# brucechin/OctopusZK

Hardware: AMD Instinct MI355X
Metric: BN254 G1 VariableBaseMSM Mscalar-mul/s at 2^20 (higher is better)
Workload: dtype u32; 1 GPU; VariableBaseMSM BN254 G1 2^20 random scalars/bases per GPU, bit-exact vs the serial CPU path (BASELINE.json configs[1]); n_per_gpu=1048576, window_bits=16, windows=8, glv=True, prepared_bases=False, msms_in_flight=3, schedule=pipeline3, parallelism=index-range shard x1, RCCL all-gather of 192-B partials + HIP point sum

## Files before the change

### include/ozk.h

```cpp
#ifndef OZK_H
#define OZK_H

#include <stddef.h>
#include <stdint.h>

#ifdef __cplusplus
extern "C" {
#endif

#define OZK_OK 0
#define OZK_E_INVALID -1
#define OZK_E_NO_DEVICE -2
#define OZK_E_NOMEM -3
#define OZK_E_INTERNAL -4

#define OZK_G1 1
#define OZK_G2 2

const char* ozk_last_error(void);
int ozk_version(void);
int ozk_device_count(void);
int ozk_device_cu_count(void);
int ozk_stream_create_cu_range(int32_t first_cu, int32_t n_cus, void** stream);
int ozk_stream_destroy(void* stream);
// ... 33 lines not shown
                            size_t* accum_ws_bytes);
int ozk_var_msm_sort_dev(const void* d_bases, int32_t prepared, const void* d_scalars, int32_t n, int32_t type,
                         void* d_sorted, size_t sorted_bytes, void* d_sort_ws, size_t sort_ws_bytes, void* stream);
int ozk_var_msm_accum_dev(const void* d_prepared, int32_t n, int32_t type, void* d_sorted, size_t sorted_bytes,
                          void* d_accum_ws, size_t accum_ws_bytes, void* d_tail, size_t tail_bytes, void* stream,
                          int32_t part);

size_t ozk_var_msm_prepared_bytes(int32_t n, int32_t type);
int ozk_var_msm_prepare_dev(const void* d_bases, int32_t n, int32_t type, void* d_prepared, size_t prepared_size,
                            void* stream);
int ozk_var_msm_prepared_dev(const void* d_prepared, const void* d_scalars, int32_t n, int32_t type, void* d_out,
                             void* d_workspace, size_t workspace_bytes, void* stream);
int ozk_bases_create_host(const uint8_t* bases, int32_t n, int32_t type, int32_t task_id, void** handle);
int ozk_var_msm_bases_host(void* handle, const uint8_t* scalars, int32_t n, uint8_t* out);
int ozk_bases_destroy(void* handle);
int ozk_bases_type(void* handle);

int ozk_order_event_create(void** ev);
int ozk_order_event_destroy(void* ev);


int ozk_points_sum_dev(const void* d_points, int32_t k, int32_t type, void* d_out, void* stream);

int ozk_groth16_combine_dev(const void* d_records, int32_t world, void* d_proof, void* stream);

int ozk_prof_enable(int on);
int ozk_prof_dominant_kernel_ms(double* avg_ms, int* launches);
int ozk_prof_dominant_kernel_stats(double* stats4, int* launches);
int ozk_prof_dominant_kernel_clock_mhz(double* stats4, int* launches);
double ozk_prof_clock_khz(void);
int ozk_var_msm_plan(int32_t n, int32_t* window_bits, int32_t* windows);
int ozk_var_msm_glv(int32_t n);
int ozk_var_msm_last_l1_path(void);

int ozk_gen_bases_dev(uint64_t seed, int32_t n, int32_t type, void* d_out_wire, void* stream);

int ozk_fixed_batch_msm_host(int32_t outerc, int32_t window_size, int32_t out_len,
                             int32_t inner_len, int32_t n, int32_t scalar_size,
                             const uint8_t* base, const uint8_t* scalars, int32_t bn_type,
                             int32_t task_id, uint8_t* out);
int ozk_fixed_double_batch_msm_host(int32_t outerc1, int32_t window_size1, int32_t outerc2,
                                    int32_t window_size2, int32_t out_len1, int32_t inner_len1,
                                    int32_t out_len2, int32_t inner_len2, int32_t n,
                                    const uint8_t* base_g1, const uint8_t* base_g2,
                                    const uint8_t* scalars, int32_t task_id, uint8_t* out);
int ozk_field_batch_mul_host(const uint8_t* in, int32_t n, int32_t task_id, uint8_t* out);

size_t ozk_fixed_batch_msm_workspace_bytes(int32_t outerc, int32_t window_size, int32_t n,
                                           int32_t bn_type);
int ozk_fixed_batch_msm_dev(int32_t outerc, int32_t window_size, int32_t n, const void* d_base,
                            const void* d_scalars, int32_t bn_type, void* d_out,
                            void* d_workspace, size_t workspace_bytes, void* stream);
int ozk_field_batch_mul_dev(const void* d_in, int32_t n, void* d_out, void* stream);
int ozk_fixed_batch_msm_compact_dev(int32_t outerc, int32_t window_size, int32_t n, const void* d_base,
                                    const void* d_scalars, int32_t bn_type, void* d_out, void* d_workspace,
                                    size_t workspace_bytes, void* stream);
int ozk_fixed_batch_msm_compact_host(int32_t outerc, int32_t window_size, int32_t n, const uint8_t* base,
                                     const uint8_t* scalars, int32_t bn_type, int32_t task_id, uint8_t* out);
int ozk_fixed_batch_msm_base_dev(int32_t outerc, int32_t window_size, int32_t n, const uint8_t* base_host,
                                 const void* d_scalars, int32_t bn_type, void* d_out, int32_t compact,
                                 void* d_workspace, size_t workspace_bytes, void* stream);

int ozk_fft_host(const uint8_t* in, int32_t n, const uint8_t* omega, int32_t task_id,
                 uint8_t* out);
size_t ozk_fft_workspace_bytes(int32_t n);
int ozk_fft_dev(const void* d_in, int32_t n, const uint8_t* omega_host32, void* d_out,
// ... 118 lines not shown
```

### octopuszk_amd/build.py

```python
import os
import shutil
import subprocess
import sys

HERE = os.path.dirname(os.path.abspath(__file__))
CSRC = os.path.join(HERE, "csrc")
ROOT = os.path.dirname(HERE)
LIB = os.path.join(HERE, "libozk_hip.so")

HIP_SOURCES = ["msm_var.hip", "msm_var_g2.hip", "msm_fixed.hip", "fft.hip", "host_ctx.hip", "pairing.hip", "msm_multi.hip",
               "point_codec.hip", "points_scale.hip", "ec_fft.hip", "points_mul.hip"]
HEADERS = ["consts_gen.h", "mad_chain_gen.h", "fp29.cuh", "fq2.cuh", "fq12.cuh", "batch_verify.cuh", "point_codec.cuh", "points_scale.cuh", "points_mul.cuh", "ec_fft.cuh", "bace.cuh", "kzg.cuh", "kzg_set.cuh", "pairing_consts_gen.h", "ec.cuh", "quad.cuh", "curve.cuh", "msm_var.cuh", "msm_var_driver.cuh", "msm_multi.cuh", "glv.cuh", "l1_whole.h", "ozk_common.h", "knobs.h", "host_ctx.h", "pin_cache.h",
           os.path.join("..", "..", "include", "ozk.h")]
HIPCC_FLAGS = ["-std=c++17", "-O3", "--offload-arch=gfx950", "-fPIC", "-fno-gpu-rdc", "-Wno-unused-result",
               "-Wno-pass-failed"]

JNI_LIBS = {
    "libAlgebraMSMVariableBaseMSM.so": "jni_var_msm.c",
    "libAlgebraMSMFixedBaseMSM.so": "jni_fixed_msm.c",
    "libAlgebraFFTAuxiliary.so": "jni_fft.c",
}


def _newer(target, deps):
    if not os.path.exists(target):
        return True
    t = os.path.getmtime(target)
    return any(os.path.exists(d) and os.path.getmtime(d) > t for d in deps)


def hipcc():
    for cand in (shutil.which("hipcc"), "/opt/rocm/bin/hipcc"):
        if cand and os.path.exists(cand):
            return cand
    raise RuntimeError("hipcc not found: the HIP library cannot be built (there is no CPU path)")


def build(force=False, verbose=True):
    srcs = [os.path.join(CSRC, s) for s in HIP_SOURCES if os.path.exists(os.path.join(CSRC, s))]
    deps = srcs + [os.path.join(CSRC, h) for h in HEADERS]
    if force or _newer(LIB, deps):
        defs = []
        if os.path.exists(os.path.join(CSRC, "fq2.cuh")):
            defs.append("-DOZK_WITH_G2")
        objdir = os.path.join(HERE, "_obj")
# ... 38 lines not shown
```

### octopuszk_amd/csrc/ec.cuh

```cuda
#pragma once
#include "fp29.cuh"

namespace ozk {

template <class EA>
struct Aff {
  EA x, y;
};

template <class CV>
struct Jac {
  typename CV::EX X;
  typename CV::EY Y;
  typename CV::EZ Z;
};

template <class CV>
OZK_HD bool is_inf(const Jac<CV>& p) { return is_zero(p.Z); }

template <class EA>
OZK_HD bool is_inf(const Aff<EA>& q) { return is_zero(q.x) && is_zero(q.y); }

template <class CV>
OZK_HD Jac<CV> from_affine(const Aff<typename CV::EA>& q) {
// ... 178 lines not shown
    Aff<typename CV::EA> qs = q;
    qs.y = typename CV::EA(reduce_to<17>(normalise(yq)));
    return xyzz_from_affine<CV>(qs);
  }
  const auto U2 = mul(q.x, p.ZZ);
  const auto S2 = mul(yq, p.ZZZ);
  const auto P = sub(U2, p.X);
  const auto R = sub(S2, p.Y);
  const auto PP = sqr(P);
  if (is_zero(PP)) {
    if (is_zero(R)) {
      Aff<typename CV::EA> qs = q;
      qs.y = typename CV::EA(reduce_to<17>(normalise(yq)));
      return xyzz_dbl_affine<CV>(qs);
    }
    Xyzz<CV> z = p;
    z.ZZ = typename CV::XZZ(el_zero(q.x));
    z.ZZZ = typename CV::XZZZ(el_zero(q.x));
    return z;
  }
  const auto PPP = mul(P, PP);
  const auto Q = mul(p.X, PP);
  const auto X3 = sub_sub2(sqr(R), PPP, Q);
  const auto Y3 = mul2(sub_nc(Q, X3), R, neg_nc(p.Y), PPP);
  Xyzz<CV> out;
  out.X = typename CV::XX(X3);
  out.Y = typename CV::XY(Y3);
  out.ZZ = typename CV::XZZ(mul(p.ZZ, PP));
  out.ZZZ = typename CV::XZZZ(mul(p.ZZZ, PPP));
  return out;
}

template <class CV>
OZK_HD Xyzz<CV> xyzz_dbl(const Xyzz<CV>& p) {
  if (is_inf(p)) return p;
  const auto U = dbl(p.Y);
  const auto V = sqr(U);
  const auto W = mul(U, V);
  const auto S = mul(p.X, V);
  const auto xx = sqr(p.X);
  const auto M = add(dbl(xx), xx);
  const auto X3 = sub(sqr(M), dbl(S));
  const auto Y3 = mulsub(M, sub(S, X3), W, p.Y);
  Xyzz<CV> r;
  r.X = typename CV::XX(X3);
  r.Y = typename CV::XY(Y3);
  r.ZZ = typename CV::XZZ(mul(V, p.ZZ));
  r.ZZZ = typename CV::XZZZ(mul(W, p.ZZZ));
  return r;
}

template <class CV>
OZK_HD Xyzz<CV> xyzz_add(const Xyzz<CV>& p, const Xyzz<CV>& q) {
  if (is_inf(q)) return p;
  if (is_inf(p)) return q;
  const auto U1 = mul(p.X, q.ZZ);
  const auto U2 = mul(q.X, p.ZZ);
  const auto S1 = mul(p.Y, q.ZZZ);
  const auto S2 = mul(q.Y, p.ZZZ);
  const auto P = sub(U2, U1);
  const auto R = sub(S2, S1);
  if (is_zero(P)) {
    if (is_zero(R)) return xyzz_dbl(p);
    Xyzz<CV> z = p;
    z.ZZ = typename CV::XZZ(el_zero(p.ZZ));
    z.ZZZ = typename CV::XZZZ(el_zero(p.ZZ));
    return z;
  }
  const auto PP = sqr(P);
  const auto PPP = mul(P, PP);
  const auto Q = mul(U1, PP);
  const auto X3 = sub(sqr(R), add(PPP, dbl(Q)));
  const auto Y3 = mulsub(R, sub(Q, X3), S1, PPP);
  Xyzz<CV> out;
  out.X = typename CV::XX(X3);
  out.Y = typename CV::XY(Y3);
  out.ZZ = typename CV::XZZ(mul(mul(p.ZZ, q.ZZ), PP));
  out.ZZZ = typename CV::XZZZ(mul(mul(p.ZZZ, q.ZZZ), PPP));
  return out;
}

template <class CV>
OZK_HD Jac<CV> xyzz_to_jac(const Xyzz<CV>& p) {
  Jac<CV> r;
  r.X = typename CV::EX(mul(p.X, p.ZZ));
  r.Y = typename CV::EY(mul(p.Y, p.ZZZ));
  r.Z = typename CV::EZ(p.ZZ);
  return r;
}

template <class CV>
OZK_HD Jac<CV> jac_add(const Jac<CV>& p, const Jac<CV>& q) {
  if (is_inf(p)) return q;
  if (is_inf(q)) return p;
  const auto& X1 = p.X;
  const auto& Y1 = p.Y;
  const auto& X2 = q.X;
  const auto& Y2 = q.Y;
  const auto Z1 = entry_reduce<32, CV>(p.Z);
  const auto Z2 = entry_reduce<32, CV>(q.Z);
  const auto Z1Z1 = sqr(Z1);
  const auto Z2Z2 = sqr(Z2);
  const auto U1 = mul(X1, Z2Z2);
  const auto U2 = mul(X2, Z1Z1);
  const auto S1 = mul(mul(Y1, Z2), Z2Z2);
  const auto S2 = mul(mul(Y2, Z1), Z1Z1);
  const auto H = sub(U2, U1);
  const auto rh = sub(S2, S1);
  if (is_zero(H)) {
    if (is_zero(rh)) return jac_dbl(p);
    return jac_infinity<CV>();
  }
  const auto I = sqr(dbl(H));
  const auto J = mul(H, I);
  const auto r = dbl(rh);
  const auto V = mul(U1, I);
  const auto X3 = sub(sqr(r), add(J, dbl(V)));
  const auto Y3 = mulsub(r, sub(V, X3), dbl(S1), J);
  const auto Z3 = mul(sub(sqr(add(Z1, Z2)), add(Z1Z1, Z2Z2)), H);
  Jac<CV> out;
// ... 42 lines not shown
```

### octopuszk_amd/csrc/fp29.cuh

```cuda
#pragma once
#include "consts_gen.h"
#include <type_traits>

#if defined(__HIPCC__)
#include <hip/hip_runtime.h>
#define OZK_HD __host__ __device__ __forceinline__
#else
#define OZK_HD inline
#endif

namespace ozk {

constexpr int ceil_div(long long a, long long b) { return (int)((a + b - 1) / b); }
constexpr int MONT_SLACK = 169;
constexpr int FE_BMAX = 16 * FE_MAXK;

template <class P, int B>
struct Fe {
  static_assert(B >= 1 && B <= FE_BMAX, "bound out of range");
  u32 l[9];
  OZK_HD Fe() {}
  template <int B2, class = std::enable_if_t<(B2 <= B)>>
  OZK_HD Fe(const Fe<P, B2>& o) {
#pragma unroll
// ... 371 lines not shown
  static_assert(B >= 1 && B <= FE_BMAX, "bound out of range");
  static_assert(LU >= 2 && LU <= 15, "limb bound out of range");
  u32 l[9];
  OZK_HD FeL() {}
  OZK_HD FeL(const Fe<P, B>& o) {
#pragma unroll
    for (int i = 0; i < 9; i++) l[i] = o.l[i];
  }
};
template <class P, int B, int LU>
OZK_HD Fe<P, B> normalise(const FeL<P, B, LU>& a) {
  Fe<P, B> r;
#pragma unroll
  for (int i = 0; i < 9; i++) r.l[i] = a.l[i];
  fe_carry(r);
  return r;
}
template <class P, int B2>
OZK_HD auto neg_nc(const Fe<P, B2>& b) {
  constexpr int K = B2 / 16 + 1;
  static_assert(K <= FE_MAXK, "sub bias table too small");
  FeL<P, neg_bound(B2), 4> r;
#pragma unroll
  for (int i = 0; i < 9; i++) r.l[i] = P::BIAS[K][i] - b.l[i];
  return r;
}
template <class P, int B1, int B2>
OZK_HD auto sub_nc(const Fe<P, B1>& a, const Fe<P, B2>& b) {
  constexpr int K = B2 / 16 + 1;
  static_assert(K <= FE_MAXK, "sub bias table too small");
  FeL<P, B1 + 16 * K, 6> r;
#pragma unroll
  for (int i = 0; i < 9; i++) r.l[i] = a.l[i] + (P::BIAS[K][i] - b.l[i]);
  return r;
}
template <class P, int B1, int B2, int B3>
OZK_HD auto sub_sub2(const Fe<P, B1>& a, const Fe<P, B2>& b, const Fe<P, B3>& c) {
  constexpr int K2 = B2 / 16 + 1, K3 = B3 / 16 + 1;
  static_assert(K2 <= FE_MAXK && K3 <= FE_MAXK, "sub bias table too small");
  Fe<P, B1 + 16 * K2 + 32 * K3> r;
#pragma unroll
  for (int i = 0; i < 9; i++) r.l[i] = a.l[i] + (P::BIAS[K2][i] - b.l[i]) + ((P::BIAS[K3][i] - c.l[i]) << 1);
  fe_carry(r);
  return r;
}
template <class P, int B1, int LU1, int B2>
OZK_HD auto select_el(bool c, const FeL<P, B1, LU1>& a, const Fe<P, B2>& b) {
  FeL<P, (B1 > B2 ? B1 : B2), LU1> r;
#pragma unroll
  for (int i = 0; i < 9; i++) r.l[i] = c ? a.l[i] : b.l[i];
  return r;
}
template <class P, int B1, int LU, int B2>
OZK_HD auto mul(const FeL<P, B1, LU>& a, const Fe<P, B2>& b) {
  static_assert(LU <= 12, "loose factor too wide for the 64-bit column accumulator");
  Fe<P, B1> an;
#pragma unroll
  for (int i = 0; i < 9; i++) an.l[i] = a.l[i];
  return mul(an, b);
}
template <class P, int B1, int LU1, int B2, int B3, int LU3, int B4>
OZK_HD auto mul2(const FeL<P, B1, LU1>& a, const Fe<P, B2>& b, const FeL<P, B3, LU3>& c, const Fe<P, B4>& d) {
  static_assert(LU1 + LU3 <= 12, "loose factors too wide for the 64-bit column accumulator");
  Fe<P, B1> an;
  Fe<P, B3> cn;
#pragma unroll
// ... 326 lines not shown
```

### octopuszk_amd/csrc/knobs.h

```cpp
#pragma once
#include <stdlib.h>
#include <string.h>

#include <atomic>
#include <mutex>

namespace ozk {

constexpr int KNOB_COMPUTED = -0x7fffffff;
constexpr int KNOB_STRING = KNOB_COMPUTED + 1;

#define OZK_KNOBS(X)                                                                                                     \
                                                   \
  X(MSM_GLV, "OZK_MSM_GLV", 1, "0: plain 256-bit windows instead of the GLV split (var MSM up to 2^23 pairs, fixed base)") \
  X(MSM_SIGNED, "OZK_MSM_SIGNED", 1, "0: unsigned window digits in the GLV form")                                        \
  X(MSM_C, "OZK_MSM_C", KNOB_COMPUTED, "window bits, 1..16 (default: the cost model's choice)")                          \
  X(MSM_L1, "OZK_MSM_L1", KNOB_COMPUTED, "sorted entries per level-1 lane (default: from the bucket size; 0 as unset)")   \
  X(MSM_L1_WHOLE, "OZK_MSM_L1_WHOLE", 1, "G1 level 1 by whole buckets on lane groups: 0 never, 1 on every plan that can take it (unset: where it pays)") \
  X(MSM_L1_ROUNDS, "OZK_MSM_L1_ROUNDS", 2, "most rounds of resident workgroups level 1 is rounded up to; 0: no rounding") \
  X(MSM_TAIL_MODE, "OZK_MSM_TAIL_MODE", -1, "0 / 1: force the latency / throughput shape of the window sums")            \
  X(MSM_SMALL_SORT, "OZK_MSM_SMALL_SORT", 1, "0: small MSMs take the two-level sort too")                                \
  X(MSM_S_LAT, "OZK_MSM_S_LAT", KNOB_COMPUTED, "buckets per lane in a latency tail's fused first level (default: 8 G1, 4 G2)") \
  X(MSM_FIN_MAX, "OZK_MSM_FIN_MAX", 4, "elements per window left to the final one-wave kernel, 1..16")                   \
                                                                                                    \
  X(HOST_SLICES, "OZK_HOST_SLICES", 8, "most slices a host-buffer MSM is cut into; 1: no slicing")                       \
  X(HOST_SLICE_MIN_LOG, "OZK_HOST_SLICE_MIN_LOG", 18, "log2 of the smallest slice")                                      \
  X(SHARD, "OZK_SHARD", 0, "1: the JNI entries shard large calls over the visible devices")                              \
  X(SHARD_MIN_N, "OZK_SHARD_MIN_N", 1 << 21, "smallest call OZK_SHARD=1 shards")                                         \
  X(SHARD_COUNT, "OZK_SHARD_COUNT", 0, "shards of such a call; 0: one per device")                                       \
  X(SHARD_RCCL, "OZK_SHARD_RCCL", 1, "0: the partials of a sharded call go through the host, not RCCL")                  \
  X(COPY_HELPERS, "OZK_COPY_HELPERS", 3, "threads staging host buffers beside the caller, 0..11 (first use only)")       \
  X(HOST_TRACE, "OZK_HOST_TRACE", 0, "1: per-call host timings on stderr; 2: with absolute timestamps")                  \
                                                                                     \
  X(FB_WS, "OZK_FB_WS", KNOB_COMPUTED, "window bits of a GLV fixed-base table (default: cost model, at most the caller's)") \
  X(FB_AFFINE, "OZK_FB_AFFINE", 1, "0: Jacobian gather-add instead of affine table records")                             \
  X(FB_TABLE_CACHE, "OZK_FB_TABLE_CACHE", 1, "0: window tables are built per call")                                      \
  X(FB_TABLE_CACHE_MB, "OZK_FB_TABLE_CACHE_MB", 1024, "MiB of cached window tables per device")                          \
  X(FB_TABLE_CACHE_SECOND_USE, "OZK_FB_TABLE_CACHE_SECOND_USE", 1, "0: a table is cached on its first use")              \
  X(FB_HOST_RANGES, "OZK_FB_HOST_RANGES", 4, "ranges a host fixed-base call downloads its results in")                   \
  X(MM_WS, "OZK_MM_WS", KNOB_COMPUTED, "window bits of the shared-base batched MSM (default: from n)")                   \
                                                                                             \
  X(FFT_MAXK, "OZK_FFT_MAXK", 8, "most butterfly stages per pass, 3..10")                                                \
  X(FFT_PLAN, "OZK_FFT_PLAN", 1, "0: stages spread evenly over the passes")                                              \
  X(FFT_KS, "OZK_FFT_KS", KNOB_STRING, "explicit stages per pass, e.g. \"8,6,8\" (must sum to log2 n)")                  \
  X(FFT_TW_PYRAMID, "OZK_FFT_TW_PYRAMID", 1, "0: twiddles from the flat table")                                          \
  X(FFT_PLAN_CACHE, "OZK_FFT_PLAN_CACHE", 1, "0: twiddle tables are built per call")                                     \
  X(FFT_PLAN_CACHE_MB, "OZK_FFT_PLAN_CACHE_MB", 4096, "MiB of cached twiddle tables per device")                         \
  X(QAP_FOLD_SCALE, "OZK_QAP_FOLD_SCALE", 1, "0: the witness map scales in a pass of its own")                           \
  X(BACE_LDS_SLOTS, "OZK_BACE_LDS_SLOTS", 16, "circuit slots kept in LDS, 0..28")

enum Knob {
#define X(id, env, dflt, doc) K_##id,
  OZK_KNOBS(X)
// ... 56 lines not shown
```

### octopuszk_amd/csrc/msm_var.cuh

```cuda
#pragma once
#include "curve.cuh"
#include "glv.cuh"
#include "l1_whole.h"

namespace ozk {

constexpr u32 BID_NONE = 0xffffffffu;

struct MsmPlan {
  int n_in;
  int glv;
  int n;
  int sd;
  int c;
  int cb;
  int W;
  int L1;
  int LK;
  int S;
  int lone;
  int small_sort;
  int S_lat;
  int fin_max;
  int tail_mode;
  int l1_whole;
  int l1_gtop;
};

OZK_HD u32 scalar_digit(const u32 (&s)[8], int w, int c) {
  const int bit = w * c;
  const int wi = bit >> 5, sh = bit & 31;
  u32 v = s[wi] >> sh;
  if (sh + c > 32 && wi + 1 < 8) v |= s[wi + 1] << (32 - sh);
  return v & ((1u << c) - 1u);
}

OZK_HD bool digit_decode(u32 code, int sd, u32& b, u32& neg) {
  if (sd) {
    const u32 t = code - 1u;
    b = t >> 1;
    neg = t & 1u;
  } else {
    b = code;
    neg = 0;
  }
  return code != 0;
}
template <class Emit>
OZK_HD void signed_digit_codes(const u32 (&e)[8], int c, int W, bool neg, Emit emit) {
  const u32 half = 1u << (c - 1);
  const u32 thr = (c == 16 && neg) ? half - 1u : half;
  u32 cy = 0;
  for (int w = 0; w < W; w++) {
    const u32 d = scalar_digit(e, w, c) + cy;
    cy = d > thr;
    const u32 m = cy ? (1u << c) - d : d;
    emit(w, (uint16_t)(m ? (((m - 1u) << 1) | (cy ^ (u32)neg)) + 1u : 0u));
// ... 1128 lines not shown
  b.ZZZ = ElemTraits<typename CV::XZZZ>::load_raw(w + 3 * RW);
  return b;
}

template <class CV>
__global__ void __launch_bounds__(256)
k_l1_whole(const uint4* __restrict__ items, const uint2* __restrict__ sent, const u32* __restrict__ pts_in,
           const u32* __restrict__ bad, WholeGeom geo, u32 n_lanes, u32* __restrict__ buckets,
           unsigned long long* __restrict__ clk) {
  using IO = CurveIO<CV>;
  using Acc = RunAcc<CV, true>;
  if (*bad != 0u) return;
  unsigned long long w0 = 0, c0 = 0;
  if (clk != nullptr && threadIdx.x == 0) {
    w0 = (unsigned long long)wall_clock64();
    c0 = (unsigned long long)clock64();
    atomicMax(&clk[0], ~w0);
  }
  const u32 t = blockIdx.x * blockDim.x + threadIdx.x;
  u32 item, g, G;
  whole_lane_map(geo, t < n_lanes ? t : 0u, &item, &g, &G);
  const bool valid = t < n_lanes && item != WHOLE_NO_ITEM;
  uint4 it = items[valid ? item : 0u];
  if (!valid) it.y = 0u;
  u32 first, n_e;
  whole_part(it.y, g, G, &first, &n_e);
  Xyzz<CV> a = xyzz_from_affine<CV>(IO::aff_infinity());
  if (n_e != 0u) {
    const u32* idx_c = reinterpret_cast<const u32*>(sent + (size_t)it.x + first);
    u32 v_cur = idx_c[0];
    u32 v_next = idx_c[n_e > 1u ? 2 : 0];
    const __amdgpu_buffer_rsrc_t table = Acc::table_rsrc(pts_in);
    typename Acc::Raw r = Acc::load_raw_buf(table, v_cur);
    for (u32 k = 0; k < n_e; k++) {
      const bool negate = (v_cur & SIDX_NEG) != 0;
      const auto q = Acc::decode_unsigned(r);
      const u32 k2 = (k + 2 < n_e) ? k + 2 : n_e - 1;
      r = Acc::load_raw_buf(table, v_next);
      v_cur = v_next;
      v_next = idx_c[2 * (size_t)k2];
      a = xyzz_madd_lazy(a, q, negate);
    }
  }
  if (__ballot(G > 1u) != 0ull) {
    const Xyzz<CV> b = xyzz_quad_swap<0xB1, CV>(a);
    if (G > 1u) a = xyzz_add(a, b);
  }
  if (__ballot(G > 2u) != 0ull) {
    const Xyzz<CV> b = xyzz_quad_swap<0x4E, CV>(a);
    if (G > 2u) a = xyzz_add(a, b);
  }
  if (g == 0u && it.y != 0u) IO::store_rec_xyzz(a, buckets + (size_t)it.z * IO::REC_WORDS);
  if (clk != nullptr && (threadIdx.x & 63) == 0) {
    const unsigned long long w1 = (unsigned long long)wall_clock64();
    atomicMax(&clk[1], w1);
    if (threadIdx.x == 0) {
      atomicAdd(&clk[2], (unsigned long long)clock64() - c0);
      atomicAdd(&clk[3], w1 - w0);
    }
  }
}

template <class CV, bool FIRSTLEVEL>
__global__ void __launch_bounds__(256)
k_wsum(const u32* __restrict__ A_in, const u32* __restrict__ R_in, const u32* __restrict__ hist,
       int m_in, int S, int g, u32* __restrict__ A_out, u32* __restrict__ R_out, int m_out, int W, int prio) {
  using IO = CurveIO<CV>;
  if (prio) __builtin_amdgcn_s_setprio(3);
  const int t = blockIdx.x * blockDim.x + threadIdx.x;
  if (t >= m_out * W) return;
  const int w = t / m_out, j = t - w * m_out;
  const size_t base = (size_t)w * m_in;
  const int lo = j * S;
// ... 66 lines not shown
  wave_combine<CV>(A, T, l, valid, g);
  if (l == 0) {
    IO::store_jac(A, A_out + ((size_t)w * m_out + j) * IO::JAC_WORDS);
    IO::store_jac(T, R_out + ((size_t)w * m_out + j) * IO::JAC_WORDS);
  }
}

template <class CV>
__global__ void __launch_bounds__(64)
k_wsum_fused(const u32* __restrict__ buckets, const u32* __restrict__ hist, int m_in, int S, int sg,
             u32* __restrict__ A_out, u32* __restrict__ R_out, int m_out, int W, int prio) {
  using IO = CurveIO<CV>;
  if (prio) __builtin_amdgcn_s_setprio(3);
  const int wave = blockIdx.x;
  if (wave >= m_out * W) return;
  const int w = wave / m_out, j = wave - w * m_out;
  const int l = threadIdx.x & 63;
  const int nseg = (m_in + S - 1) / S;
  int valid = nseg - j * 64;
  if (valid > 64) valid = 64;
  const size_t base = (size_t)w * m_in;
  const int lo = (j * 64 + l) * S;
  int hi = lo + S;
  if (hi > m_in) hi = m_in;
  Jac<CV> run = jac_infinity<CV>(), ws = jac_infinity<CV>();
  for (int e = hi - 1; e >= lo; e--) {
    if (hist[base + e] != 0) run = jac_add(run, IO::load_rec(buckets + (base + e) * IO::REC_WORDS));
    if (e > lo) ws = jac_add(ws, run);
  }
  wave_combine<CV>(ws, run, l, valid, sg);
  if (l == 0) {
    IO::store_jac(ws, A_out + ((size_t)w * m_out + j) * IO::JAC_WORDS);
    IO::store_jac(run, R_out + ((size_t)w * m_out + j) * IO::JAC_WORDS);
  }
}

struct SliceBuckets {
  const u32* buckets[16];
  const u32* hist[16];
};
template <class CV>
__global__ void __launch_bounds__(256) k_bucket_combine(SliceBuckets t, int K, u32* __restrict__ buckets0,
                                                        u32* __restrict__ hist0, size_t NB) {
  using IO = CurveIO<CV>;
  const size_t e = (size_t)blockIdx.x * blockDim.x + threadIdx.x;
  if (e >= NB) return;
  bool have = hist0[e] != 0, changed = false;
  Jac<CV> acc = jac_infinity<CV>();
  if (have) acc = IO::load_rec(buckets0 + e * IO::REC_WORDS);
  for (int k = 1; k < K; k++) {
    if (t.hist[k][e] == 0) continue;
    acc = jac_add(acc, IO::load_rec(t.buckets[k] + e * IO::REC_WORDS));
    changed = true;
  }
  if (changed) {
    IO::store_rec_jac(acc, buckets0 + e * IO::REC_WORDS);
    hist0[e] = 1;
  }
}

template <class CV>
__device__ __forceinline__ void write_normalised_inline(const Jac<CV>& r, u32* out) {
  CurveIO<CV>::template write<WireOut>(r, out);
}
template <class CV>
__device__ void write_normalised(const Jac<CV>& r, u32* out) {
// ... 140 lines not shown
```

### octopuszk_amd/csrc/msm_var.hip

```cpp
#include "msm_var_driver.cuh"

#include <dlfcn.h>
#include <rccl/rccl.h>

#include <algorithm>
#include <chrono>
#include <new>
#include <string>
#include <thread>
#include <vector>

OZK_G2_DRIVER_INSTANCES(extern)

using namespace ozk;

template <class F>
static auto with_plan(int n, int type, F f) {
  return by_point_type(type, [&](auto t) { return f(t, plan_for<typename decltype(t)::CV>(n, false)); });
}
#define CV_OF(t) typename decltype(t)::CV

extern "C" {

size_t ozk_var_msm_workspace_bytes(int32_t n, int32_t type) {
// ... 743 lines not shown
  *launches = (int)m.size();
  if (m.empty()) return OZK_OK;
  std::sort(m.begin(), m.end());
  stats4[0] = tot / (double)m.size();
  stats4[1] = m[m.size() / 2];
  stats4[2] = m.front();
  stats4[3] = m.back();
  return OZK_OK;
}

double ozk_prof_clock_khz(void) { return g_prof.clk_khz; }

int ozk_var_msm_plan(int32_t n, int32_t* window_bits, int32_t* windows) {
  if (n <= 0 || !window_bits || !windows) return fail(OZK_E_INVALID, "bad argument");
  const MsmPlan p = make_plan(n);
  *window_bits = p.c;
  *windows = p.W;
  return OZK_OK;
}

int ozk_var_msm_glv(int32_t n) { return n > 0 ? make_plan(n).glv : 0; }

int ozk_var_msm_last_l1_path(void) {
  const L1PathLast& last = g_l1_path_last;
  if (last.planned <= 0) return last.planned;
  u32 bad = 0;
  if (hipDeviceSynchronize() != hipSuccess || hipMemcpy(&bad, last.d_bad, sizeof(bad), hipMemcpyDeviceToHost) != hipSuccess) {
    (void)hipGetLastError();
    return -1;
  }
  return bad ? 0 : 1;
}

const char* ozk_last_error(void) { return err_buf(); }
int ozk_version(void) { return 2; }
int ozk_device_count(void) {
  int n = 0;
  if (hipGetDeviceCount(&n) != hipSuccess) return 0;
  return n;
}

}
```

### octopuszk_amd/csrc/msm_var_driver.cuh

```cuda
#pragma once
#include <hip/hip_ext.h>
#include <pthread.h>
#include <stdlib.h>

#include <atomic>
#include <vector>

#include "msm_var.cuh"
#include "host_ctx.h"
#include "fq2.cuh"

namespace ozk {

enum { PROF_OFF = 0, PROF_EVENTS = 1, PROF_CLOCK = 2 };
struct ProfState {
  pthread_mutex_t mu = PTHREAD_MUTEX_INITIALIZER;
  std::atomic<int> mode{PROF_OFF};
  int src = PROF_EVENTS;
  int every = 1, seen = 0;
  int count = 0;
  std::vector<hipEvent_t> e0, e1;
  bool created = false;
  int ev_device = -1;
  unsigned long long* d_clk = nullptr;
// ... 73 lines not shown
  p.sd = sd_ok && c >= 2;
  p.cb = c - p.sd;
  p.W = ((p.glv ? 128 : 256) + c - 1) / c;
  {
    const long long per_bucket = (long long)p.n >> p.cb;
    long long l1 = per_bucket * 5 / 16;
    long long l1_min = p.n >= (1 << 20) ? 52 : 40;
    if (p.glv) {
      const long long cap = (long long)p.n * p.W;
      long long fit = cap / 65536;
      const int top_bits = 127 - (p.W - 1) * p.c;
      const int tb = top_bits - p.sd;
      const long long per_top = (top_bits >= 1 && top_bits < p.c) ? ((long long)p.n >> (tb > 0 ? tb : 0)) : per_bucket;
      const long long pieces = (per_top + 9) / 10;
      if (fit < pieces) fit = pieces;
      if (fit < 8) fit = 8;
      if (fit < l1_min) l1_min = fit;
    }
    if (l1 < l1_min) l1 = l1_min;
    if (l1 > 1024) l1 = 1024;
    p.L1 = knob_or(K_MSM_L1, (int)l1);
  }
  if (p.L1 < 2) p.L1 = 2;
  p.LK = PLAN_LK;
  p.S = PLAN_S;
  p.lone = 0;
  p.small_sort = p.n <= SORTS_MAX_N && p.cb <= SORTS_MAX_CB && knob(K_MSM_SMALL_SORT) != 0;
  p.S_lat = p.S;
  p.fin_max = knob(K_MSM_FIN_MAX);
  if (p.fin_max < 1) p.fin_max = 1;
  if (p.fin_max > 16) p.fin_max = 16;
  p.tail_mode = knob(K_MSM_TAIL_MODE);
  if (p.tail_mode != 0 && p.tail_mode != 1) p.tail_mode = -1;
  p.l1_whole = 0;
  p.l1_gtop = WHOLE_G;
  return p;
}

template <class CV>
static MsmPlan plan_for(int n, bool lone) {
  MsmPlan p = make_plan(n);
  p.lone = lone;
  const long long max_rounds = knob(K_MSM_L1_ROUNDS);
  bool rounded = false;
  if ((CV::LDS_ACC || lone) && knob_or(K_MSM_L1, 0) == 0 && max_rounds != 0) {
    static int cu_count = 0;
    if (cu_count == 0) {
      int dev = 0, cus = 0;
      if (hipGetDevice(&dev) == hipSuccess && hipDeviceGetAttribute(&cus, hipDeviceAttributeMultiprocessorCount, dev) == hipSuccess &&
          cus > 0)
        cu_count = cus;
      else
        cu_count = 256;
    }
    const int slots = (CV::LDS_ACC ? 2 : 3) * cu_count;
    const long long cap = (long long)p.n * p.W;
    const long long blocks = ((cap + p.L1 - 1) / p.L1 + 255) / 256;
    long long rounds = blocks / slots > 0 ? blocks / slots : 1;
    if (rounds > max_rounds) rounds = max_rounds;
    long long l1 = (cap + 256LL * slots * rounds - 1) / (256LL * slots * rounds);
    if (l1 > p.L1 && l1 <= 1024) {
      p.L1 = (int)l1;
      rounded = true;
    }
  }
  const int s_lat = knob_or(K_MSM_S_LAT, std::is_same<CV, G1Cfg>::value && p.cb >= 13 ? 8 : p.S);
// ... 285 lines not shown
    lanes = (n_in + p.LK - 1) / p.LK;
    if (!first_generic && (int)lanes <= SMALL_LEVEL_LANES) {
      hipLaunchKernelGGL((k_segreduce_small<CT>), dim3(1), dim3(TB), 0, st, L.total + 1, (int)n_in, p.LK, L.buckets,
                         L.slot_bid[cur], L.slot_pts[cur], L.slot_bid[cur ^ 1], L.slot_pts[cur ^ 1]);
      break;
    }
    hipLaunchKernelGGL((k_segreduce<CT, false>), dim3((unsigned)((lanes + TB - 1) / TB)), dim3(TB), 0, st,
                       first_generic ? L.slot_bid2 : L.slot_bid[cur], (const u32*)nullptr, L.slot_pts[cur],
                       L.total + 1, (int)n_in, p.LK, L.buckets, L.slot_bid[cur ^ 1], L.slot_pts[cur ^ 1], (int)lanes,
                       (unsigned long long*)nullptr);
    first_generic = false;
    if (lanes == 1) break;
    n_in = 2 * lanes;
    cur ^= 1;
  }
  OZK_HIP(hipGetLastError());
  return OZK_OK;
}

template <class CV>
int var_msm_head(const MsmPlan& p, const void* d_bases, const void* d_scalars, void* ws, size_t ws_bytes, void* tail,
                        size_t tail_bytes, hipStream_t st, hipEvent_t order_ev = nullptr,
                        const void* prepared = nullptr) {
  const RegionBytes rb = region_bytes<CV>(p);
  if (rb.sorted + rb.sort_ws + rb.accum_ws > ws_bytes)
    return fail(OZK_E_INVALID, "workspace too small: need %zu bytes, got %zu", rb.sorted + rb.sort_ws + rb.accum_ws,
                ws_bytes);
  uint8_t* w = (uint8_t*)ws;
  int rc = var_msm_sort<CV>(p, d_bases, d_scalars, w, rb.sorted, w + rb.sorted, rb.sort_ws, st, order_ev, prepared);
  if (rc) return rc;
  return var_msm_accum<CV>(p, w, rb.sorted, w + rb.sorted + rb.sort_ws, rb.accum_ws, tail, tail_bytes, st, prepared);
}

template <class CV>
int var_msm_tail(const MsmPlan& p, void* tail, size_t tail_bytes, void* d_out, hipStream_t st,
                        hipEvent_t order_ev = nullptr, int mode = TAIL_LATENCY) {
  hip_clear_stale();
  using CT = CV;
  MsmLayout L;
  const size_t tneed = tail_layout<CV>(p, L, tail, tail_bytes);
  if (tneed > tail_bytes) return fail(OZK_E_INVALID, "tail buffer too small: need %zu bytes, got %zu", tneed, tail_bytes);
  const int shape = p.tail_mode >= 0 ? p.tail_mode : mode;
  const bool fused = shape == TAIL_LATENCY;
  const int S0 = fused && mode == TAIL_LATENCY ? p.S_lat : p.S;
  launch_wsum0<CV>(p, L, st, S0, fused);
  int m_in, g, k = 0;
  first_level_shape(p, S0, fused, &m_in, &g);
  const int TB = 256;
  const int sg = ilog2((uint32_t)p.S);
  while (shape == TAIL_THROUGHPUT && m_in > TAIL_SERIAL_ABOVE) {
    const int m_out = (m_in + p.S - 1) / p.S;
    const int tot = m_out * p.W;
    hipLaunchKernelGGL((k_wsum<CT, false>), dim3((tot + TB - 1) / TB), dim3(TB), 0, st, L.wA[k], L.wR[k],
                       (const u32*)nullptr, m_in, p.S, g, L.wA[k ^ 1], L.wR[k ^ 1], m_out, p.W, 1);
    m_in = m_out;
    g += sg;
    k ^= 1;
  }
  if (order_ev) OZK_HIP(hipEventRecord(order_ev, st));
  while (m_in > p.fin_max) {
    const int m_out = (m_in + 63) / 64;
    const int tot = m_out * p.W;
    hipLaunchKernelGGL((k_wsum_wave<CT>), dim3(tot), dim3(64), 0, st, L.wA[k], L.wR[k], m_in, g, L.wA[k ^ 1],
                       L.wR[k ^ 1], m_out, p.W);
    m_in = m_out;
    g += 6;
    k ^= 1;
  }
  hipLaunchKernelGGL((k_finalize<CT>), dim3(1), dim3(64), 0, st, L.wA[k], L.wR[k], m_in, g, p.W, p.c, p.sd,
                     (u32*)d_out);
  OZK_HIP(hipGetLastError());
  return OZK_OK;
}

template <class CV>
// ... 273 lines not shown
```

### octopuszk_amd/lib.py

```python
import ctypes
import os

HERE = os.path.dirname(os.path.abspath(__file__))
LIB_PATH = os.environ.get("OZK_LIB_PATH") or os.path.join(HERE, "libozk_hip.so")

_lib = None

c_u8p = ctypes.POINTER(ctypes.c_uint8)
i32 = ctypes.c_int32
vp = ctypes.c_void_p
sz = ctypes.c_size_t

_SIGS = {
    "ozk_last_error": (ctypes.c_char_p, []),
    "ozk_version": (ctypes.c_int, []),
    "ozk_device_count": (ctypes.c_int, []),
    "ozk_var_msm_host": (ctypes.c_int, [vp, vp, i32, i32, i32, vp]),
    "ozk_var_double_msm_host": (ctypes.c_int, [vp, vp, vp, i32, i32, vp]),
    "ozk_var_msm_sharded_host": (ctypes.c_int, [vp, vp, i32, i32, i32, vp]),
    "ozk_var_msm_auto_host": (ctypes.c_int, [vp, vp, i32, i32, i32, vp]),
    "ozk_var_double_msm_sharded_host": (ctypes.c_int, [vp, vp, vp, i32, i32, vp]),
    "ozk_var_double_msm_auto_host": (ctypes.c_int, [vp, vp, vp, i32, i32, vp]),
    "ozk_shard_last_exchange": (ctypes.c_int, []),
    "ozk_shard_comms_release": (None, []),
    "ozk_var_msm_workspace_bytes": (sz, [i32, i32]),
    "ozk_var_msm_dev": (ctypes.c_int, [vp, vp, i32, i32, vp, vp, sz, vp]),
    "ozk_prof_enable": (ctypes.c_int, [ctypes.c_int]),
    "ozk_prof_dominant_kernel_ms": (ctypes.c_int, [ctypes.POINTER(ctypes.c_double), ctypes.POINTER(ctypes.c_int)]),
    "ozk_prof_dominant_kernel_stats": (ctypes.c_int, [ctypes.POINTER(ctypes.c_double), ctypes.POINTER(ctypes.c_int)]),
    "ozk_prof_clock_khz": (ctypes.c_double, []),
    "ozk_prof_dominant_kernel_clock_mhz": (ctypes.c_int, [ctypes.POINTER(ctypes.c_double), ctypes.POINTER(ctypes.c_int)]),
    "ozk_var_msm_plan": (ctypes.c_int, [i32, ctypes.POINTER(i32), ctypes.POINTER(i32)]),
    "ozk_var_msm_glv": (ctypes.c_int, [i32]),
    "ozk_var_msm_last_l1_path": (ctypes.c_int, []),
    "ozk_gen_bases_dev": (ctypes.c_int, [ctypes.c_uint64, i32, i32, vp, vp]),
    "ozk_var_msm_stage_bytes": (ctypes.c_int, [i32, i32, ctypes.POINTER(sz), ctypes.POINTER(sz), ctypes.POINTER(sz)]),
    "ozk_var_msm_sort_dev": (ctypes.c_int, [vp, i32, vp, i32, i32, vp, sz, vp, sz, vp]),
    "ozk_var_msm_accum_dev": (ctypes.c_int, [vp, i32, i32, vp, sz, vp, sz, vp, sz, vp, i32]),
    "ozk_device_cu_count": (ctypes.c_int, []),
    "ozk_stream_create_cu_range": (ctypes.c_int, [i32, i32, ctypes.POINTER(ctypes.c_void_p)]),
    "ozk_stream_destroy": (ctypes.c_int, [vp]),
    "ozk_var_msm_head_workspace_bytes": (sz, [i32, i32]),
    "ozk_var_msm_tail_bytes": (sz, [i32, i32]),
    "ozk_var_msm_head_dev": (ctypes.c_int, [vp, i32, vp, i32, i32, vp, sz, vp, sz, vp, vp]),
    "ozk_var_msm_tail_dev": (ctypes.c_int, [i32, i32, vp, sz, vp, vp, vp, i32]),
    "ozk_bases_create_host": (ctypes.c_int, [vp, i32, i32, i32, ctypes.POINTER(vp)]),
    "ozk_var_msm_bases_host": (ctypes.c_int, [vp, vp, i32, vp]),
    "ozk_bases_destroy": (ctypes.c_int, [vp]),
    "ozk_var_msm_prepared_bytes": (sz, [i32, i32]),
    "ozk_var_msm_prepare_dev": (ctypes.c_int, [vp, i32, i32, vp, sz, vp]),
    "ozk_var_msm_prepared_dev": (ctypes.c_int, [vp, vp, i32, i32, vp, vp, sz, vp]),
    "ozk_order_event_create": (ctypes.c_int, [ctypes.POINTER(vp)]),
    "ozk_order_event_destroy": (ctypes.c_int, [vp]),
    "ozk_points_sum_dev": (ctypes.c_int, [vp, i32, i32, vp, vp]),
    "ozk_groth16_combine_dev": (ctypes.c_int, [vp, i32, vp, vp]),
    "ozk_fixed_batch_msm_host": (ctypes.c_int, [i32, i32, i32, i32, i32, i32, vp, vp, i32, i32, vp]),
    "ozk_fixed_double_batch_msm_host": (ctypes.c_int, [i32] * 9 + [vp, vp, vp, i32, vp]),
    "ozk_field_batch_mul_host": (ctypes.c_int, [vp, i32, i32, vp]),
    "ozk_fixed_batch_msm_workspace_bytes": (sz, [i32, i32, i32, i32]),
    "ozk_fixed_batch_msm_dev": (ctypes.c_int, [i32, i32, i32, vp, vp, i32, vp, vp, sz, vp]),
    "ozk_field_batch_mul_dev": (ctypes.c_int, [vp, i32, vp, vp]),
    "ozk_fixed_batch_msm_compact_dev": (ctypes.c_int, [i32, i32, i32, vp, vp, i32, vp, vp, sz, vp]),
    "ozk_fixed_batch_msm_compact_host": (ctypes.c_int, [i32, i32, i32, vp, vp, i32, i32, vp]),
    "ozk_fixed_batch_msm_base_dev": (ctypes.c_int, [i32, i32, i32, vp, vp, i32, vp, i32, vp, sz, vp]),
    "ozk_fft_compact_host": (ctypes.c_int, [vp, i32, vp, i32, vp]),
    "ozk_fft_compact_dev": (ctypes.c_int, [vp, i32, vp, vp, vp, sz, vp]),
    "ozk_tuning_reload": (ctypes.c_int, []),
# ... 98 lines not shown
```

Baseline: 742.6 Mscalar-mul/s.

## Add row/column window-sum tail and cheaper first bucket additions

Result: faster. 751.4 Mscalar-mul/s, median of 6 (+1.2%).

```diff
diff --git a/include/ozk.h b/include/ozk.h
--- a/include/ozk.h
+++ b/include/ozk.h
@@ -89,6 +89,7 @@
 int ozk_var_msm_plan(int32_t n, int32_t* window_bits, int32_t* windows);
 int ozk_var_msm_glv(int32_t n);
 int ozk_var_msm_last_l1_path(void);
+int ozk_var_msm_last_tail_form(void);
 
 int ozk_gen_bases_dev(uint64_t seed, int32_t n, int32_t type, void* d_out_wire, void* stream);
 
diff --git a/octopuszk_amd/build.py b/octopuszk_amd/build.py
--- a/octopuszk_amd/build.py
+++ b/octopuszk_amd/build.py
@@ -10,7 +10,7 @@
 
 HIP_SOURCES = ["msm_var.hip", "msm_var_g2.hip", "msm_fixed.hip", "fft.hip", "host_ctx.hip", "pairing.hip", "msm_multi.hip",
                "point_codec.hip", "points_scale.hip", "ec_fft.hip", "points_mul.hip"]
-HEADERS = ["consts_gen.h", "mad_chain_gen.h", "fp29.cuh", "fq2.cuh", "fq12.cuh", "batch_verify.cuh", "point_codec.cuh", "points_scale.cuh", "points_mul.cuh", "ec_fft.cuh", "bace.cuh", "kzg.cuh", "kzg_set.cuh", "pairing_consts_gen.h", "ec.cuh", "quad.cuh", "curve.cuh", "msm_var.cuh", "msm_var_driver.cuh", "msm_multi.cuh", "glv.cuh", "l1_whole.h", "ozk_common.h", "knobs.h", "host_ctx.h", "pin_cache.h",
+HEADERS = ["consts_gen.h", "mad_chain_gen.h", "fp29.cuh", "fq2.cuh", "fq12.cuh", "batch_verify.cuh", "point_codec.cuh", "points_scale.cuh", "points_mul.cuh", "ec_fft.cuh", "bace.cuh", "kzg.cuh", "kzg_set.cuh", "pairing_consts_gen.h", "ec.cuh", "quad.cuh", "curve.cuh", "msm_var.cuh", "msm_var_driver.cuh", "msm_multi.cuh", "glv.cuh", "l1_whole.h", "wsum_rc.h", "ozk_common.h", "knobs.h", "host_ctx.h", "pin_cache.h",
            os.path.join("..", "..", "include", "ozk.h")]
 HIPCC_FLAGS = ["-std=c++17", "-O3", "--offload-arch=gfx950", "-fPIC", "-fno-gpu-rdc", "-Wno-unused-result",
                "-Wno-pass-failed"]
diff --git a/octopuszk_amd/csrc/ec.cuh b/octopuszk_amd/csrc/ec.cuh
--- a/octopuszk_amd/csrc/ec.cuh
+++ b/octopuszk_amd/csrc/ec.cuh
@@ -234,6 +234,52 @@
 }
 
 template <class CV>
+OZK_HD Xyzz<CV> xyzz_from_affine_signed(const Aff<typename CV::EA>& q, bool negate) {
+  if (is_inf(q)) return xyzz_from_affine<CV>(q);
+  Aff<typename CV::EA> qs = q;
+  qs.y = typename CV::EA(reduce_to<17>(normalise(select_el(negate, neg_nc(q.y), q.y))));
+  return xyzz_from_affine<CV>(qs);
+}
+
+template <class CV>
+OZK_HD Xyzz<CV> xyzz_add_affine2_lazy(const Xyzz<CV>& p, const Aff<typename CV::EA>& q, bool negate) {
+  if (is_inf(q)) return p;
+  if (is_inf(p)) return xyzz_from_affine_signed<CV>(q, negate);
+  using EA = typename CV::EA;
+  EA X1, Y1;
+#pragma unroll
+  for (int i = 0; i < 9; i++) {
+    X1.l[i] = p.X.l[i];
+    Y1.l[i] = p.Y.l[i];
+  }
+  const auto yq = select_el(negate, neg_nc(q.y), q.y);
+  const auto P = sub(q.x, X1);
+  const auto R = sub(yq, Y1);
+  const auto PP = sqr(P);
+  if (is_zero(PP)) {
+    if (is_zero(R)) {
+      Aff<EA> qs = q;
+      qs.y = EA(reduce_to<17>(normalise(yq)));
+      return xyzz_dbl_affine<CV>(qs);
+    }
+    Xyzz<CV> z = p;
+    z.ZZ = typename CV::XZZ(el_zero(q.x));
+    z.ZZZ = typename CV::XZZZ(el_zero(q.x));
+    return z;
+  }
+  const auto PPP = mul(P, PP);
+  const auto Q = mul(X1, PP);
+  const auto X3 = sub_sub2(sqr(R), PPP, Q);
+  const auto Y3 = mul2(sub_nc(Q, X3), R, neg_nc(Y1), PPP);
+  Xyzz<CV> out;
+  out.X = typename CV::XX(X3);
+  out.Y = typename CV::XY(Y3);
+  out.ZZ = typename CV::XZZ(PP);
+  out.ZZZ = typename CV::XZZZ(PPP);
+  return out;
+}
+
+template <class CV>
 OZK_HD Xyzz<CV> xyzz_dbl(const Xyzz<CV>& p) {
   if (is_inf(p)) return p;
   const auto U = dbl(p.Y);
@@ -288,6 +334,17 @@
   r.X = typename CV::EX(mul(p.X, p.ZZ));
   r.Y = typename CV::EY(mul(p.Y, p.ZZZ));
   r.Z = typename CV::EZ(p.ZZ);
+  return r;
+}
+
+template <class CV>
+OZK_HD Xyzz<CV> jac_to_xyzz(const Jac<CV>& p) {
+  const auto zz = sqr(p.Z);
+  Xyzz<CV> r;
+  r.X = typename CV::XX(p.X);
+  r.Y = typename CV::XY(reduce_to<52>(p.Y));
+  r.ZZ = typename CV::XZZ(reduce_to<17>(zz));
+  r.ZZZ = typename CV::XZZZ(reduce_to<17>(mul(zz, p.Z)));
   return r;
 }
 
diff --git a/octopuszk_amd/csrc/fp29.cuh b/octopuszk_amd/csrc/fp29.cuh
--- a/octopuszk_amd/csrc/fp29.cuh
+++ b/octopuszk_amd/csrc/fp29.cuh
@@ -427,6 +427,17 @@
   FeL<P, B1 + 16 * K, 6> r;
 #pragma unroll
   for (int i = 0; i < 9; i++) r.l[i] = a.l[i] + (P::BIAS[K][i] - b.l[i]);
+  return r;
+}
+template <class P, int B1, int LU, int B2>
+OZK_HD auto sub(const FeL<P, B1, LU>& a, const Fe<P, B2>& b) {
+  constexpr int K = B2 / 16 + 1;
+  static_assert(K <= FE_MAXK, "sub bias table too small");
+  static_assert(LU <= 11, "loose minuend too wide for a 32-bit limb");
+  Fe<P, B1 + 16 * K> r;
+#pragma unroll
+  for (int i = 0; i < 9; i++) r.l[i] = a.l[i] + (P::BIAS[K][i] - b.l[i]);
+  fe_carry(r);
   return r;
 }
 template <class P, int B1, int B2, int B3>
diff --git a/octopuszk_amd/csrc/knobs.h b/octopuszk_amd/csrc/knobs.h
--- a/octopuszk_amd/csrc/knobs.h
+++ b/octopuszk_amd/csrc/knobs.h
@@ -19,6 +19,7 @@
   X(MSM_L1_WHOLE, "OZK_MSM_L1_WHOLE", 1, "G1 level 1 by whole buckets on lane groups: 0 never, 1 on every plan that can take it (unset: where it pays)") \
   X(MSM_L1_ROUNDS, "OZK_MSM_L1_ROUNDS", 2, "most rounds of resident workgroups level 1 is rounded up to; 0: no rounding") \
   X(MSM_TAIL_MODE, "OZK_MSM_TAIL_MODE", -1, "0 / 1: force the latency / throughput shape of the window sums")            \
+  X(MSM_TAIL_RC, "OZK_MSM_TAIL_RC", -1, "1: G1 throughput window sums by bucket rows and columns wherever the buffers take them (0 / unset: the serial levels)") \
   X(MSM_SMALL_SORT, "OZK_MSM_SMALL_SORT", 1, "0: small MSMs take the two-level sort too")                                \
   X(MSM_S_LAT, "OZK_MSM_S_LAT", KNOB_COMPUTED, "buckets per lane in a latency tail's fused first level (default: 8 G1, 4 G2)") \
   X(MSM_FIN_MAX, "OZK_MSM_FIN_MAX", 4, "elements per window left to the final one-wave kernel, 1..16")                   \
diff --git a/octopuszk_amd/csrc/msm_var.cuh b/octopuszk_amd/csrc/msm_var.cuh
--- a/octopuszk_amd/csrc/msm_var.cuh
+++ b/octopuszk_amd/csrc/msm_var.cuh
@@ -2,6 +2,7 @@
 #include "curve.cuh"
 #include "glv.cuh"
 #include "l1_whole.h"
+#include "wsum_rc.h"
 
 namespace ozk {
 
@@ -23,6 +24,7 @@
   int S_lat;
   int fin_max;
   int tail_mode;
+  int tail_rc;
   int l1_whole;
   int l1_gtop;
 };
@@ -1217,13 +1219,26 @@
     u32 v_next = idx_c[n_e > 1u ? 2 : 0];
     const __amdgpu_buffer_rsrc_t table = Acc::table_rsrc(pts_in);
     typename Acc::Raw r = Acc::load_raw_buf(table, v_cur);
-    for (u32 k = 0; k < n_e; k++) {
-      const bool negate = (v_cur & SIDX_NEG) != 0;
+    bool negate;
+    auto take = [&](u32 k) {
+      negate = (v_cur & SIDX_NEG) != 0;
       const auto q = Acc::decode_unsigned(r);
       const u32 k2 = (k + 2 < n_e) ? k + 2 : n_e - 1;
       r = Acc::load_raw_buf(table, v_next);
       v_cur = v_next;
       v_next = idx_c[2 * (size_t)k2];
+      return q;
+    };
+    {
+      const auto q = take(0u);
+      a = xyzz_from_affine_signed<CV>(q, negate);
+    }
+    if (n_e > 1u) {
+      const auto q = take(1u);
+      a = xyzz_add_affine2_lazy(a, q, negate);
+    }
+    for (u32 k = 2; k < n_e; k++) {
+      const auto q = take(k);
       a = xyzz_madd_lazy(a, q, negate);
     }
   }
@@ -1356,6 +1371,91 @@
   if (l == 0) {
     IO::store_jac(ws, A_out + ((size_t)w * m_out + j) * IO::JAC_WORDS);
     IO::store_jac(run, R_out + ((size_t)w * m_out + j) * IO::JAC_WORDS);
+  }
+}
+
+template <class CV>
+__device__ __forceinline__ Xyzz<CV> load_rec_as_xyzz(const u32* p) {
+  using IO = CurveIO<CV>;
+  if (p[IO::REC_TAG] == IO::TAG_JAC) return jac_to_xyzz<CV>(IO::load_jac(p));
+  return IO::load_xyzz(p);
+}
+
+template <class CV>
+__global__ void __launch_bounds__(256)
+k_rc_partial(const u32* __restrict__ buckets, const u32* __restrict__ hist, RcGeom geo, int W,
+             u32* __restrict__ row_out, u32* __restrict__ col_out) {
+  using IO = CurveIO<CV>;
+  const int per = rc_partial_lanes(geo);
+  const int t = blockIdx.x * blockDim.x + threadIdx.x;
+  if (t >= per * W) return;
+  const int w = t / per, i = t - w * per;
+  const size_t base = (size_t)w << geo.cb;
+#pragma unroll 1
+  for (int pass = 0; pass < 2; pass++) {
+    const int slots = pass ? rc_col_slots(geo) : rc_row_slots(geo);
+    if (i >= slots) continue;
+    u32 first;
+    int n;
+    if (pass) rc_col_part(geo, i, RC_CHUNK, &first, &n);
+    else rc_row_part(geo, i, RC_CHUNK, &first, &n);
+    const u32 stride = pass ? (u32)geo.cols : 1u;
+    Xyzz<CV> a = xyzz_from_affine<CV>(IO::aff_infinity());
+#pragma unroll 1
+    for (int k = 0; k < n; k++) {
+      const size_t b = base + first + (size_t)k * stride;
+      if (hist[b] != 0) a = xyzz_add(a, load_rec_as_xyzz<CV>(buckets + b * IO::REC_WORDS));
+    }
+    IO::store_rec_xyzz(a, (pass ? col_out : row_out) + ((size_t)w * slots + i) * IO::REC_WORDS);
+  }
+}
+
+template <class CV>
+__global__ void __launch_bounds__(256)
+k_rc_reduce(const u32* __restrict__ row_in, const u32* __restrict__ col_in, RcGeom geo, int W,
+            u32* __restrict__ A_out, u32* __restrict__ R_out) {
+  using IO = CurveIO<CV>;
+  __builtin_amdgcn_s_setprio(3);
+  const int m = geo.cols;
+  const int t = blockIdx.x * blockDim.x + threadIdx.x;
+  if (t >= 2 * m * W) return;
+  const int v = t / m, e = t - v * m;
+  const int w = v >> 1, list = v & 1;
+  Xyzz<CV> a = xyzz_from_affine<CV>(IO::aff_infinity());
+  if (list == 1 || e < geo.rows) {
+    int col, first, stride, n;
+    rc_reduce_part(geo, list ? geo.rows + e : e, &col, &first, &stride, &n);
+    const u32* src = (col ? col_in : row_in) + (size_t)w * (col ? rc_col_slots(geo) : rc_row_slots(geo)) * IO::REC_WORDS;
+#pragma unroll 1
+    for (int k = 0; k < n; k++) a = xyzz_add(a, IO::load_xyzz(src + (size_t)(first + k * stride) * IO::REC_WORDS));
+  }
+  IO::store_jac(jac_infinity<CV>(), A_out + (size_t)t * IO::JAC_WORDS);
+  IO::store_jac(xyzz_to_jac(a), R_out + (size_t)t * IO::JAC_WORDS);
+}
+
+template <class CV>
+__global__ void __launch_bounds__(64)
+k_rc_wave(const u32* __restrict__ A_in, const u32* __restrict__ R_in, int m_in, int g_row, int g_col,
+          u32* __restrict__ A_out, u32* __restrict__ R_out, int m_out, int lists) {
+  using IO = CurveIO<CV>;
+  __builtin_amdgcn_s_setprio(3);
+  const int wave = blockIdx.x;
+  if (wave >= m_out * lists) return;
+  const int v = wave / m_out, j = wave - v * m_out;
+  const int l = threadIdx.x & 63;
+  const int e = j * 64 + l;
+  int valid = m_in - j * 64;
+  if (valid > 64) valid = 64;
+  Jac<CV> A = jac_infinity<CV>(), T = jac_infinity<CV>();
+  if (e < m_in) {
+    A = IO::load_jac(A_in + ((size_t)v * m_in + e) * IO::JAC_WORDS);
+    T = IO::load_jac(R_in + ((size_t)v * m_in + e) * IO::JAC_WORDS);
+  }
+  wave_combine<CV>(A, T, l, valid, (v & 1) ? g_col : g_row);
+  if (l == 0) {
+    if (m_out == 1 && (v & 1)) T = jac_infinity<CV>();
+    IO::store_jac(A, A_out + ((size_t)v * m_out + j) * IO::JAC_WORDS);
+    IO::store_jac(T, R_out + ((size_t)v * m_out + j) * IO::JAC_WORDS);
   }
 }
 
diff --git a/octopuszk_amd/csrc/msm_var.hip b/octopuszk_amd/csrc/msm_var.hip
--- a/octopuszk_amd/csrc/msm_var.hip
+++ b/octopuszk_amd/csrc/msm_var.hip
@@ -799,6 +799,8 @@
   return bad ? 0 : 1;
 }
 
+int ozk_var_msm_last_tail_form(void) { return g_tail_form_last; }
+
 const char* ozk_last_error(void) { return err_buf(); }
 int ozk_version(void) { return 2; }
 int ozk_device_count(void) {
diff --git a/octopuszk_amd/csrc/msm_var_driver.cuh b/octopuszk_amd/csrc/msm_var_driver.cuh
--- a/octopuszk_amd/csrc/msm_var_driver.cuh
+++ b/octopuszk_amd/csrc/msm_var_driver.cuh
@@ -129,6 +129,8 @@
   if (p.fin_max > 16) p.fin_max = 16;
   p.tail_mode = knob(K_MSM_TAIL_MODE);
   if (p.tail_mode != 0 && p.tail_mode != 1) p.tail_mode = -1;
+  p.tail_rc = knob(K_MSM_TAIL_RC);
+  if (p.tail_rc != 1) p.tail_rc = 0;
   p.l1_whole = 0;
   p.l1_gtop = WHOLE_G;
   return p;
@@ -480,6 +482,41 @@
   return var_msm_accum<CV>(p, w, rb.sorted, w + rb.sorted + rb.sort_ws, rb.accum_ws, tail, tail_bytes, st, prepared);
 }
 
+inline thread_local int g_tail_form_last = -1;
+template <class CV>
+bool tail_rc_applies(const MsmPlan& p, const MsmLayout& L) {
+  using IO = CurveIO<CV>;
+  if (p.tail_rc != 1) return false;
+  const RcGeom geo = rc_geom(p.cb);
+  const size_t have = L.m1 * IO::JAC_WORDS;
+  return (size_t)rc_row_slots(geo) * IO::REC_WORDS <= have && (size_t)rc_col_slots(geo) * IO::REC_WORDS <= have &&
+         (size_t)2 * geo.cols * IO::JAC_WORDS <= have;
+}
+template <class CV>
+int var_msm_tail_rc(const MsmPlan& p, const MsmLayout& L, void* d_out, hipStream_t st, hipEvent_t order_ev) {
+  const int TB = 256;
+  const RcGeom geo = rc_geom(p.cb);
+  const int lanes1 = rc_partial_lanes(geo) * p.W, lanes2 = 2 * geo.cols * p.W;
+  hipLaunchKernelGGL((k_rc_partial<CV>), dim3((lanes1 + TB - 1) / TB), dim3(TB), 0, st, (const u32*)L.buckets,
+                     (const u32*)L.hist_t, geo, p.W, L.wA[0], L.wR[0]);
+  hipLaunchKernelGGL((k_rc_reduce<CV>), dim3((lanes2 + TB - 1) / TB), dim3(TB), 0, st, (const u32*)L.wA[0],
+                     (const u32*)L.wR[0], geo, p.W, L.wA[1], L.wR[1]);
+  if (order_ev) OZK_HIP(hipEventRecord(order_ev, st));
+  int m_in = geo.cols, g_row = geo.s, g_col = 0, k = 1;
+  while (m_in > 1) {
+    const int m_out = (m_in + 63) / 64;
+    hipLaunchKernelGGL((k_rc_wave<CV>), dim3(m_out * 2 * p.W), dim3(64), 0, st, (const u32*)L.wA[k], (const u32*)L.wR[k],
+                       m_in, g_row, g_col, L.wA[k ^ 1], L.wR[k ^ 1], m_out, 2 * p.W);
+    m_in = m_out;
+    g_row += 6;
+    g_col += 6;
+    k ^= 1;
+  }
+  hipLaunchKernelGGL((k_finalize<CV>), dim3(1), dim3(64), 0, st, L.wA[k], L.wR[k], 2, 0, p.W, p.c, p.sd, (u32*)d_out);
+  OZK_HIP(hipGetLastError());
+  return OZK_OK;
+}
+
 template <class CV>
 int var_msm_tail(const MsmPlan& p, void* tail, size_t tail_bytes, void* d_out, hipStream_t st,
                         hipEvent_t order_ev = nullptr, int mode = TAIL_LATENCY) {
@@ -489,6 +526,13 @@
   const size_t tneed = tail_layout<CV>(p, L, tail, tail_bytes);
   if (tneed > tail_bytes) return fail(OZK_E_INVALID, "tail buffer too small: need %zu bytes, got %zu", tneed, tail_bytes);
   const int shape = p.tail_mode >= 0 ? p.tail_mode : mode;
+  g_tail_form_last = 0;
+  if constexpr (std::is_same<CV, G1Cfg>::value) {
+    if (shape == TAIL_THROUGHPUT && tail_rc_applies<CV>(p, L)) {
+      g_tail_form_last = 1;
+      return var_msm_tail_rc<CV>(p, L, d_out, st, order_ev);
+    }
+  }
   const bool fused = shape == TAIL_LATENCY;
   const int S0 = fused && mode == TAIL_LATENCY ? p.S_lat : p.S;
   launch_wsum0<CV>(p, L, st, S0, fused);
diff --git a/octopuszk_amd/csrc/wsum_rc.h b/octopuszk_amd/csrc/wsum_rc.h
--- /dev/null
+++ b/octopuszk_amd/csrc/wsum_rc.h
@@ -0,0 +1,69 @@
+#pragma once
+#include <stdint.h>
+
+#if !defined(OZK_HD)
+#if defined(__HIPCC__)
+#include <hip/hip_runtime.h>
+#define OZK_HD __host__ __device__ __forceinline__
+#else
+#define OZK_HD inline
+#endif
+#endif
+
+namespace ozk {
+
+constexpr int RC_CHUNK = 16;
+
+struct RcGeom {
+  int cb;
+  int s;
+  int rows;
+  int cols;
+  int row_parts;
+  int col_parts;
+};
+OZK_HD RcGeom rc_geom(int cb, int s, int chunk) {
+  RcGeom g;
+  g.cb = cb;
+  g.s = s;
+  g.rows = 1 << (cb - s);
+  g.cols = 1 << s;
+  g.row_parts = (g.cols + chunk - 1) / chunk;
+  g.col_parts = (g.rows + chunk - 1) / chunk;
+  return g;
+}
+OZK_HD RcGeom rc_geom(int cb) { return rc_geom(cb, (cb + 1) / 2, RC_CHUNK); }
+OZK_HD int rc_row_slots(const RcGeom& g) { return g.rows * g.row_parts; }
+OZK_HD int rc_col_slots(const RcGeom& g) { return g.cols * g.col_parts; }
+OZK_HD int rc_partial_lanes(const RcGeom& g) {
+  return rc_row_slots(g) > rc_col_slots(g) ? rc_row_slots(g) : rc_col_slots(g);
+}
+OZK_HD int rc_reduce_lanes(const RcGeom& g) { return g.rows + g.cols; }
+
+OZK_HD void rc_row_part(const RcGeom& g, int t, int chunk, uint32_t* first, int* n) {
+  const int r = t / g.row_parts, k = t - r * g.row_parts;
+  const int q0 = k * chunk;
+  *first = ((uint32_t)r << g.s) + (uint32_t)q0;
+  *n = g.cols - q0 < chunk ? g.cols - q0 : chunk;
+}
+OZK_HD void rc_col_part(const RcGeom& g, int t, int chunk, uint32_t* first, int* n) {
+  const int k = t >> g.s, q = t & (g.cols - 1);
+  const int r0 = k * chunk;
+  *first = ((uint32_t)r0 << g.s) + (uint32_t)q;
+  *n = g.rows - r0 < chunk ? g.rows - r0 : chunk;
+}
+OZK_HD void rc_reduce_part(const RcGeom& g, int u, int* col, int* first, int* stride, int* n) {
+  if (u < g.rows) {
+    *col = 0;
+    *first = u * g.row_parts;
+    *stride = 1;
+    *n = g.row_parts;
+  } else {
+    *col = 1;
+    *first = u - g.rows;
+    *stride = g.cols;
+    *n = g.col_parts;
+  }
+}
+
+}
diff --git a/octopuszk_amd/lib.py b/octopuszk_amd/lib.py
--- a/octopuszk_amd/lib.py
+++ b/octopuszk_amd/lib.py
@@ -33,6 +33,7 @@
     "ozk_var_msm_plan": (ctypes.c_int, [i32, ctypes.POINTER(i32), ctypes.POINTER(i32)]),
     "ozk_var_msm_glv": (ctypes.c_int, [i32]),
     "ozk_var_msm_last_l1_path": (ctypes.c_int, []),
+    "ozk_var_msm_last_tail_form": (ctypes.c_int, []),
     "ozk_gen_bases_dev": (ctypes.c_int, [ctypes.c_uint64, i32, i32, vp, vp]),
     "ozk_var_msm_stage_bytes": (ctypes.c_int, [i32, i32, ctypes.POINTER(sz), ctypes.POINTER(sz), ctypes.POINTER(sz)]),
     "ozk_var_msm_sort_dev": (ctypes.c_int, [vp, i32, vp, i32, i32, vp, sz, vp, sz, vp]),
```
